# lxtGH/Video-K-Net

Hardware: AMD Instinct MI355X
Metric: frames/sec (S=3, N=100, 1024x2048) (higher is better)
Workload: dtype f32; 1 GPU; cfg2 video_knet_s3_r50: VideoKernelIterHead S=3, N=100 proposals + 17 stuff = 117 kernels, C=256, 1024x2048 frame -> 128x256 stride-8 features, ffn tracking link, x4 bilinear upsample of the final logits; streams_per_gpu=1, parallelism=frame-sharded dp1, x_storage=fp32

## Files before the change

include/vkn.h:

```cpp
#ifndef VKN_H
#define VKN_H
#include <stddef.h>
#include <stdint.h>

#ifdef __cplusplus
extern "C" {
#endif

#define VKN_VERSION 0x000600

#define VKN_OK 0
#define VKN_E_ARG (-1)
#define VKN_E_SHAPE (-2)
#define VKN_E_WORKSPACE (-3)
#define VKN_E_LAUNCH (-4)
#define VKN_E_ALIGN (-5)
#define VKN_E_RANGE (-6)

#define VKN_STATUS_RANGE 1u

#define VKN_FLAG_REF_KERNELS 1u
#define VKN_FLAG_EXACT_GEMM 2u
#define VKN_FLAG_LOGITS_HANDOFF 4u
#define VKN_FLAG_BITS_HANDOFF 16u
#define VKN_X_F32 0
#define VKN_X_F16 1
#define VKN_X_BF16 2
#define VKN_FLAG_X_F16 64u
#define VKN_FLAG_X_BF16 128u
#define VKN_FLAG_CHAIN_LAUNCHES 256u
#define VKN_FLAG_CHAIN_PERSISTENT 512u
#define VKN_FLAG_JOIN_EARLY 32768u
#define VKN_FLAG_LINK_RESERVE 262144u
#define VKN_FLAG_LINK_NO_RESERVE 524288u
#define VKN_FLAG_SCALED_F16 16384u
#define VKN_FLAG_CHAIN_BF16X3 65536u
#define VKN_FLAG_CHAIN_KSPLIT 8192u
#define VKN_FLAG_SERIAL_LINK 32u
#define VKN_FLAG_CLIP_LINK 8u

#define VKN_FLAG_INIT_SEPARATE 131072u
#define VKN_FLAG_PHASE_A 1024u
#define VKN_FLAG_PHASE_B 2048u
#define VKN_FLAG_PHASE_C 4096u
#define VKN_FLAG_PHASE_MASK (VKN_FLAG_PHASE_A | VKN_FLAG_PHASE_B | VKN_FLAG_PHASE_C)

#define VKN_MAX_FCS 4

typedef struct VknDims {
    int B;
    int N;
    int C;
    int H, W;
    int heads;
    int ff;
    int ncls;
// ... 359 lines not shown
```

video-k-net_amd/csrc/vkn_api.hip:

```cpp
#include "../../include/vkn.h"
#include "../../include/vkn_decode.h"
#include "vkn_common.h"
#include "vkn_launch.h"

namespace {

struct Carver {
    char* base;
    size_t off;
    template <class T>
    T* take(size_t n) {
        off = (off + 255) & ~(size_t)255;
        T* p = base ? reinterpret_cast<T*>(base + off) : nullptr;
        off += n * sizeof(T);
        return p;
    }
};

inline bool aligned16(const void* p) { return (reinterpret_cast<uintptr_t>(p) & 15) == 0; }
inline int npt_of(int N) { return (N + 31) / 32 * 32; }

struct StageWs {
    float *part, *cntp, *xraw, *cnt, *xfeat, *params, *inputf, *ig, *ug, *f, *obj1, *qkv, *ao, *obj2, *h, *partial, *t1, *t2,
        *maskfeat, *kb, *kern32, *lq, *lkv, *lobj, *lupd, *lf;
    _Float16 *kfh, *kfl;
    int* status;
};


enum MasksFrom {
    FROM_LOGITS,
    FROM_BITS,
    FROM_GATHERED,
    FROM_XFEAT
};
enum MasksTo {
    TO_LOGITS,
    TO_BITS,
    TO_GATHER,
    TO_KERNELS,
    TO_NONE
};
struct StageCall {
    const VknStageWeights* w = nullptr;
    const float *x = nullptr, *obj_in = nullptr;
    float *obj_out = nullptr, *cls_logits = nullptr, *x_feat_out = nullptr;
    bool cls_sigmoid = false;
    MasksFrom from = FROM_LOGITS;
    const float *masks_in = nullptr, *xfeat_in = nullptr;
    const unsigned* bits_in = nullptr;
    MasksTo to = TO_LOGITS;
    float* masks_out = nullptr;
    unsigned* bits_out = nullptr;
    float *kern_out = nullptr, *kb_out = nullptr;
    hipEvent_t prof0 = nullptr, prof1 = nullptr, obj_ready = nullptr;
    float* up_out = nullptr;
    int up_stride = 0, up_chunk = 0;
    bool* up_done = nullptr;
    int link_reserve = 0;
    const float* prev_obj = nullptr;
    float* track_out = nullptr;
    const VknStageWeights* link_pre = nullptr;
    const float* prev_pre = nullptr;
    const VknStageWeights* link_track = nullptr;
// ... 597 lines not shown
    const bool pre_link = c.link_pre && c.prev_pre;
    const bool need_xfeat = (pre_link && c.link_pre->dyn_w) || (c.link_track && c.track_src == 1) || c.keep_xfeat;
    if (xdt_of(flags) && !chain_only && (ref || (P % 64) != 0)) return VKN_E_SHAPE;
    PrepW pw;
    VKN_TRY(carve_pw(d, w, flags, &pw));
    const bool comp = pw.dynft != nullptr;
    const bool fewrow = comp && chain_ks_ok(d, w, pw, flags, have_cls), persistent = comp && chain_fast_ok(d, w, pw, flags, have_cls);
    const bool fast = fewrow || persistent;

    const bool will_fast = !given_xfeat && persistent && vkn_dbg_env("VKN_CHAIN_TOUCH", 1);
    const void* touch_nx = vkn_dbg_env("VKN_CHAIN_TOUCH", 1) ? c.touch_next : nullptr;
    const size_t touch_nx_bytes = touch_nx ? c.touch_next_bytes : 0;
    if (c.from == FROM_LOGITS || c.from == FROM_BITS)
        VKN_TRY(run_gather(d, c.x, c.masks_in, c.from == FROM_BITS ? c.bits_in : nullptr, s, flags, st, will_fast ? w->prepared : nullptr,
                           will_fast ? w->prepared_bytes : 0));

    float* xfeat = c.x_feat_out ? c.x_feat_out : s.xfeat;
    VknEpi e = mk_epi(d);
    if (given_xfeat) {
        xfeat = const_cast<float*>(c.xfeat_in);
    } else if (has_ft) {
        if (!comp || c.x_feat_out || need_xfeat) {
            e.bias = w->ft_b; e.rowscale = s.cnt; e.out = xfeat; e.ldo = C;
            VKN_TRY(vkn_launch_gemm(s.xraw, nullptr, C, w->ft_w, pw.ft, M, C, C, 1, nullptr, e, st));
        }
    } else {
        if (hipMemcpyAsync(xfeat, s.xraw, (size_t)M * C * sizeof(float), hipMemcpyDeviceToDevice, st) != hipSuccess)
            return VKN_E_LAUNCH;
    }

// ... 344 lines not shown
        return VKN_E_ALIGN;
    const int nstuff = cat_stuff ? ncls - num_thing_classes : 0, N = Np + nstuff;
    if (C % 32 != 0 || C > 256 || Np > 256 || ncls > 256) return VKN_E_SHAPE;
    InitWs s;
    const size_t need = carve_init(B, Np, ncls, C, P, sem && !seg_preds, nullptr, &s);
    if (!ws || ws_bytes < need || !aligned16(ws)) return VKN_E_WORKSPACE;
    carve_init(B, Np, ncls, C, P, sem && !seg_preds, static_cast<char*>(ws), &s);
    hipStream_t st = static_cast<hipStream_t>(stream);
    const bool ref = (flags & VKN_FLAG_REF_KERNELS) != 0, ref_decode = ref || (P & 1);
    const int xdt = xdt_of(flags);
    if (xdt && (ref || (P % 64) != 0 || with_obj == 2)) return VKN_E_SHAPE;
    const size_t xes = xdt ? 2 : 4;

    const bool one_pass = sem && !ref && !xdt && with_obj != 2 && s.ph && !(flags & VKN_FLAG_INIT_SEPARATE) &&
                          vkn_init_pass_supported(Np, ncls, C, P) != 0;
    const float* xf = loc_feats;
    if (one_pass) {
        VKN_TRY(vkn_launch_split_planes(init_w, s.ph, s.pl, 1, Np, C, st));
        VKN_TRY(vkn_launch_split_planes(seg_w, s.ph + (size_t)Np * C, s.pl + (size_t)Np * C, 1, ncls, C, st));
        InitPassArgs a{};
        a.loc = loc_feats; a.sem = sem_feats; a.kh = s.ph; a.kl = s.pl; a.seg_b = seg_b; a.x_out = x_feats; a.masks = mask_preds;
        a.seg = seg_preds; a.bits = with_obj ? s.bits : nullptr; a.thr = thr_logit; a.Np = Np; a.ncls = ncls; a.nth = num_thing_classes;
        a.cat = nstuff > 0 ? 1 : 0; a.N = N; a.C = C; a.P = P; a.npt = npt_of(Np);
        VKN_TRY(vkn_launch_init_pass(a, B, st));
        xf = x_feats;
    } else {
        if (ref_decode) {
            VKN_TRY(vkn_launch_decode_ref_ex(loc_feats, init_w, nullptr, mask_preds, B, Np, C, P, 1, N, st));
        } else {
            VKN_TRY(vkn_launch_split_planes(init_w, s.ih, s.il, 1, Np, C, st));
// ... 15 lines not shown
            }
            if (xdt) VKN_TRY(vkn_launch_add2_half(sem_feats, loc_feats, x_feats, (size_t)B * C * P, xdt, st));
            else VKN_TRY(vkn_launch_add2(sem_feats, loc_feats, x_feats, (size_t)B * C * P, st));
            xf = x_feats;
        } else if (x_feats && x_feats != loc_feats) {
            if (hipMemcpyAsync(x_feats, loc_feats, (size_t)B * C * P * xes, hipMemcpyDeviceToDevice, st) != hipSuccess)
                return VKN_E_LAUNCH;
        }
    }
    const float* obj = nullptr;
    if (with_obj) {
        if (with_obj == 2) {
            if (ref) return VKN_E_SHAPE;
            VKN_TRY(vkn_launch_gather_soft(xf, mask_preds, thr_logit, s.obj, s.cnt, s.part, s.cntp, B, Np, C, P, N, st));
        } else if (ref) VKN_TRY(vkn_launch_gather_ref_ex(xf, mask_preds, thr_logit, s.obj, s.cnt, B, Np, C, P, N, st));
        else if (one_pass) VKN_TRY(vkn_launch_gather_bits(xf, s.bits, s.obj, s.cnt, s.part, s.cntp, B, Np, C, P, st));
        else VKN_TRY(vkn_launch_gather_ex(xf, mask_preds, thr_logit, s.obj, s.cnt, s.part, s.cntp, B, Np, C, P, N, st, xdt));
        obj = s.obj;
    }
    return vkn_launch_init_finish(init_w, obj, seg_w, proposal_feats, B, Np, N, num_thing_classes, C, st);
}

size_t vkn_sizeof_panoptic_cfg(void) { return sizeof(VknPanopticCfg); }

size_t vkn_panoptic_workspace_bytes(const VknPanopticCfg* cfg, int B, int N) {
    if (!cfg || B <= 0 || N <= 0 || cfg->num_proposals > N || cfg->max_per_img <= 0) return 0;
    return vkn_panoptic_ws_bytes(B, cfg->max_per_img + (N - cfg->num_proposals), cfg->Ho, cfg->Wo);
}

int vkn_panoptic_joint_f32(const VknPanopticCfg* cfg, const float* cls_prob, const float* mask_logits, int B, int N, int ncls,
                           int* panoptic_seg, int* info, int* nseg, int* bbox, void* ws, size_t ws_bytes, void* stream) {
    if (!cfg || !cls_prob || !mask_logits || !panoptic_seg || !info || !nseg || B <= 0 || N <= 0 || ncls <= 0) return VKN_E_ARG;
    if (!ws || !aligned16(ws)) return VKN_E_WORKSPACE;
    return vkn_launch_panoptic_joint(cfg, cls_prob, mask_logits, B, N, ncls, panoptic_seg, info, nseg, bbox, ws, ws_bytes,
                                     static_cast<hipStream_t>(stream));
// ... 367 lines not shown
    StageWs s;
    float *mtmp, *otmp, *ctmp;
    unsigned* bits[2];
    const size_t need = carve_head(d, nullptr, &s, &mtmp, &otmp, &ctmp, bits);
    if (!ws || ws_bytes < need || !aligned16(ws)) return VKN_E_WORKSPACE;
    carve_head(d, static_cast<char*>(ws), &s, &mtmp, &otmp, &ctmp, bits);
    hipStream_t st = static_cast<hipStream_t>(stream);
    const bool use_bits = !(flags & (VKN_FLAG_REF_KERNELS | VKN_FLAG_LOGITS_HANDOFF)) && ((d->H * d->W) % 64) == 0;
    const bool use_fused = use_bits && !(flags & VKN_FLAG_BITS_HANDOFF) && vkn_fused_supported(d->C, d->H * d->W);

    const unsigned ph = flags & VKN_FLAG_PHASE_MASK;
    const bool do_a = !ph || (ph & VKN_FLAG_PHASE_A), do_b = !ph || (ph & VKN_FLAG_PHASE_B), do_c = !ph || (ph & VKN_FLAG_PHASE_C);
    if (ph && !(link_pre && (flags & VKN_FLAG_CLIP_LINK) && prev_obj)) return VKN_E_ARG;

    const int link_reserve = (flags & VKN_FLAG_LINK_NO_RESERVE) ? 0 : ((flags & VKN_FLAG_LINK_RESERVE) ? 2 : 1);
    const float* m_in = mask_preds_in;
    const float* o_in = proposal_feats;
    SideStream* joined = nullptr;
    bool up_done = false;
    for (int sidx = 0; sidx < num_stages; ++sidx) {
        const bool last = (sidx == num_stages - 1);
        if (!last && !do_a) {
            const bool to_out_s = ((num_stages - 1 - sidx) & 1) == 0;
            m_in = to_out_s ? mask_preds_out : mtmp;
            o_in = to_out_s ? obj_out : otmp;
            continue;
        }
        const bool to_out = ((num_stages - 1 - sidx) & 1) == 0;
        float* m_out = to_out ? mask_preds_out : mtmp;
        float* o_out = to_out ? obj_out : otmp;
// ... 1 lines not shown
        const bool clip = prev && (flags & VKN_FLAG_CLIP_LINK);
        SideStream* side = (prev && !(flags & VKN_FLAG_SERIAL_LINK)) ? side_stream() : nullptr;
        const bool link_after = clip || side;
        const float* prev_in_stage = link_after ? nullptr : prev;
        const unsigned* b_in = (use_bits && !use_fused && sidx > 0) ? bits[(sidx - 1) & 1] : nullptr;
        unsigned* b_out = (use_bits && !use_fused && !last) ? bits[sidx & 1] : nullptr;
        const float* prev_pre = (last && link_pre) ? prev_obj : nullptr;
        const bool seq = prev_pre && (flags & VKN_FLAG_CLIP_LINK) && (d->B > 1 || ph);
        const VknStageWeights* ltrack = (last && track_out) ? link_track : nullptr;
        StageCall c{};
        c.w = &stages[sidx]; c.x = x; c.obj_in = o_in; c.obj_out = o_out;
        c.cls_logits = last ? cls_prob : ctmp;
        c.cls_sigmoid = last;
        c.from = (use_fused && sidx > 0) ? FROM_GATHERED : (b_in ? FROM_BITS : FROM_LOGITS);
        c.masks_in = m_in; c.bits_in = b_in;
        c.link_pre = prev_pre ? link_pre : nullptr; c.prev_pre = prev_pre;
        c.link_track = ltrack; c.track_src = track_src;
        if (!last && use_fused && !(flags & (VKN_FLAG_CHAIN_LAUNCHES | VKN_FLAG_EXACT_GEMM)) && stages[sidx + 1].prepared) {
            PrepW pwn;
            (void)carve_pw(d, &stages[sidx + 1], flags, &pwn);
            if ((flags & VKN_FLAG_CHAIN_PERSISTENT) || (d->B * d->N + 31) / 32 >= persistent_min_row_tiles(pwn, flags)) {
                if (chain_h2(pwn, flags, false)) {
                    c.touch_next = pwn.h2[VKN_H2_DYNFT];
                    c.touch_next_bytes = (size_t)(reinterpret_cast<const char*>(pwn.h2_scale) - static_cast<const char*>(pwn.h2[VKN_H2_DYNFT]));
                } else {
                    c.touch_next = stages[sidx + 1].prepared;
                    c.touch_next_bytes = stages[sidx + 1].prepared_bytes;
                }
            }
        }
// ... 70 lines not shown
```

video-k-net_amd/csrc/vkn_common.h:

```cpp
#pragma once
#include <hip/hip_runtime.h>
#include <stdint.h>

typedef _Float16 half8 __attribute__((ext_vector_type(8)));
typedef _Float16 half4 __attribute__((ext_vector_type(4)));
typedef float f32x16 __attribute__((ext_vector_type(16)));
typedef float f32x4 __attribute__((ext_vector_type(4)));
typedef float f32x2 __attribute__((ext_vector_type(2)));

#define VKN_WAVE 64

#ifdef VKN_DEBUG
#include <stdlib.h>
static inline int vkn_dbg_env(const char* name, int dflt) {
    const char* e = getenv(name);
    return e ? atoi(e) : dflt;
}
#else
#define vkn_dbg_env(name, dflt) (dflt)
#endif
#ifdef VKN_DEBUG
#define VKN_ABL_IS(param, k) ((param) == (k))
#else
#define VKN_ABL_IS(param, k) false
// ... 40 lines not shown
    VKN_DPP_STEP(fmaxf, v, 0x143, 0xC, ninf);
    return __uint_as_float((unsigned)__builtin_amdgcn_readlane((int)__float_as_uint(v), 63));
}
#undef VKN_DPP_STEP

#define VKN_OK 0
#define VKN_E_ARG (-1)
#define VKN_E_SHAPE (-2)
#define VKN_E_WORKSPACE (-3)
#define VKN_E_LAUNCH (-4)
#define VKN_E_ALIGN (-5)
#define VKN_E_RANGE (-6)
#ifndef VKN_STATUS_RANGE
#define VKN_STATUS_RANGE 1
#endif

static inline int vkn_allow_full_lds(const void* fn, unsigned long long* done_mask) {
    int dev = 0;
    if (hipGetDevice(&dev) != hipSuccess) return -1;
    const unsigned long long bit = 1ull << (dev & 63);
    if (__atomic_load_n(done_mask, __ATOMIC_ACQUIRE) & bit) return 0;
    hipFuncAttributes fa;
    if (hipFuncGetAttributes(&fa, fn) != hipSuccess) return -1;
    const int dyn = 160 * 1024 - (int)fa.sharedSizeBytes;
    if (hipFuncSetAttribute(fn, hipFuncAttributeMaxDynamicSharedMemorySize, dyn) != hipSuccess) return -1;
    __atomic_fetch_or(done_mask, bit, __ATOMIC_RELEASE);
    return 0;
}
#define VKN_ALLOW_FULL_LDS(fn)                                                        \
    do {                                                                              \
// ... 9 lines not shown
```

video-k-net_amd/csrc/vkn_gather.hip:

```cpp
#include "vkn_common.h"
#include "vkn_launch.h"

#define GA_THREADS 512
#define GA_WAVES 8
#define GA_PT 32
#define GA_LDR 40

template <int NB, int BITS, int XH = 0>
__global__ __launch_bounds__(GA_THREADS, 2) void k_gather_mfma(const float* __restrict__ x,
                                                               const float* __restrict__ masks, float thr,
                                                               float* __restrict__ part, float* __restrict__ cntp, int N,
                                                               int NPT, int n0, int C, int P, int px_per_wg,
                                                               long long mask_fs, int ileave, int x_alias) {
    extern __shared__ __attribute__((aligned(16))) char smem[];
    constexpr bool REAL = (BITS == 2 || BITS == 3);
    static_assert(!(XH && REAL), "half-storage x: binary operands only");
    constexpr int XCH = XH ? 2 : 4;
    const int rows_buf = 2 * C + (REAL ? 2 : 1) * NB * 32;
    _Float16* lds = reinterpret_cast<_Float16*>(smem);

    const int b = blockIdx.y, gidx = blockIdx.x, G = gridDim.x;
    const int tid = threadIdx.x, lane = tid & 63;
    const int wave = __builtin_amdgcn_readfirstlane(tid >> 6);
    const int g = lane >> 5, li = lane & 31;
// ... 479 lines not shown
        xraw[((size_t)b * N + n) * C + c] = s;
    }
    if (threadIdx.x == 0) {
        float s = 0.f;
        for (int p = 0; p < P; ++p)
            if (mp[p] >= thr) s += 1.f;
        cnt[(size_t)b * N + n] = s;
    }
}

int vkn_launch_gather_reduce(const float* part, const float* cntp, float* xraw, float* cnt, int B, int N, int C, int G,
                             hipStream_t stream, int* status, const void* touch, size_t touch_bytes) {
    if (touch_bytes >= (1ull << 31)) touch = nullptr;
    hipLaunchKernelGGL(k_gather_reduce, dim3(B * N), dim3(256), 0, stream, part, cntp, xraw, cnt, N, (N + 31) / 32 * 32, C, G, status,
                       static_cast<const char*>(touch), (unsigned)touch_bytes);
    VKN_CHECK_LAUNCH();
    return VKN_OK;
}

int vkn_gather_groups(int B, int P) {
    int wg_per_frame = 256 / (B > 0 ? B : 1);
    if (wg_per_frame < 1) wg_per_frame = 1;
    int px_per_wg = (P + wg_per_frame - 1) / wg_per_frame;
    px_per_wg = (px_per_wg + GA_PT - 1) / GA_PT * GA_PT;
    return (P + px_per_wg - 1) / px_per_wg;
}

int vkn_launch_gather(const float* x, const float* masks, float thr, float* xraw, float* cnt, float* part, float* cntp,
                      int B, int N, int C, int P, hipStream_t stream, int xdt, int* status, const void* touch, size_t touch_bytes) {
    return vkn_launch_gather_ex(x, masks, thr, xraw, cnt, part, cntp, B, N, C, P, N, stream, xdt, status, touch, touch_bytes);
// ... 122 lines not shown
```

video-k-net_amd/csrc/vkn_init.hip:

```cpp
#include <hip/hip_runtime.h>

#include "vkn_common.h"
#include "vkn_launch.h"

__global__ __launch_bounds__(256) void k_add2(const float* __restrict__ a, const float* __restrict__ b,
                                              float* __restrict__ out, size_t n4, size_t n) {
    const size_t stride = (size_t)gridDim.x * blockDim.x;
    for (size_t i = (size_t)blockIdx.x * blockDim.x + threadIdx.x; i < n4; i += stride) {
        const f32x4 va = __builtin_nontemporal_load(reinterpret_cast<const f32x4*>(a) + i);
        const f32x4 vb = __builtin_nontemporal_load(reinterpret_cast<const f32x4*>(b) + i);
        reinterpret_cast<f32x4*>(out)[i] = va + vb;
    }
    for (size_t i = n4 * 4 + (size_t)blockIdx.x * blockDim.x + threadIdx.x; i < n; i += stride) out[i] = a[i] + b[i];
}

int vkn_launch_add2(const float* a, const float* b, float* out, size_t n, hipStream_t st) {
    const bool vec = ((reinterpret_cast<uintptr_t>(a) | reinterpret_cast<uintptr_t>(b) | reinterpret_cast<uintptr_t>(out)) & 15) == 0;
    const size_t n4 = vec ? n / 4 : 0;
    size_t blocks = (n4 + 255) / 256;
    if (blocks > 8192) blocks = 8192;
    if (blocks < 1) blocks = 1;
    hipLaunchKernelGGL(k_add2, dim3((unsigned)blocks), dim3(256), 0, st, a, b, out, n4, n);
    VKN_CHECK_LAUNCH();
    return VKN_OK;
// ... 27 lines not shown
    const bool vec = ((reinterpret_cast<uintptr_t>(a) | reinterpret_cast<uintptr_t>(b) | reinterpret_cast<uintptr_t>(out)) & 15) == 0;
    const size_t n8 = vec ? n / 8 : 0;
    size_t blocks = (n8 + 255) / 256;
    if (blocks > 8192) blocks = 8192;
    if (blocks < 1) blocks = 1;
    const unsigned short *pa = static_cast<const unsigned short*>(a), *pb = static_cast<const unsigned short*>(b);
    unsigned short* po = static_cast<unsigned short*>(out);
    if (xdt == 1) hipLaunchKernelGGL(k_add2h<1>, dim3((unsigned)blocks), dim3(256), 0, st, pa, pb, po, n8, n);
    else hipLaunchKernelGGL(k_add2h<2>, dim3((unsigned)blocks), dim3(256), 0, st, pa, pb, po, n8, n);
    VKN_CHECK_LAUNCH();
    return VKN_OK;
}

__global__ __launch_bounds__(64) void k_init_finish(const float* __restrict__ init_w, const float* __restrict__ obj,
                                                    const float* __restrict__ seg_w, float* __restrict__ out, int Np, int N,
                                                    int nth, int C) {
    const int row = blockIdx.x;
    const int b = row / N, n = row - b * N;
    for (int c = threadIdx.x; c < C; c += 64) {
        float v;
        if (n < Np) {
            v = init_w[(size_t)n * C + c];
            if (obj) v += obj[((size_t)b * Np + n) * C + c];
        } else {
            v = seg_w[(size_t)(nth + n - Np) * C + c];
        }
        out[(size_t)row * C + c] = v;
    }
}

int vkn_launch_init_finish(const float* init_w, const float* obj, const float* seg_w, float* out, int B, int Np, int N, int nth,
                           int C, hipStream_t st) {
    hipLaunchKernelGGL(k_init_finish, dim3(B * N), dim3(64), 0, st, init_w, obj, seg_w, out, Np, N, nth, C);
    VKN_CHECK_LAUNCH();
    return VKN_OK;
}

typedef unsigned int ip_u32x2 __attribute__((ext_vector_type(2)));
#define IP_THREADS 512
#define IP_WAVES 8
#define IP_TILE 64

template <int NB, int SLO>
__device__ __forceinline__ void ip_store_tile(const f32x16 (&acc)[2][NB], const InitPassArgs& A, __amdgpu_buffer_rsrc_t mrs,
                                              __amdgpu_buffer_rsrc_t srs, int p0, int li, int g, int Ntot) {
    int Pq = A.P;
    asm volatile("" : "+s"(Pq));
    const int vst = ((4 * g) * Pq + 2 * li) << 2;
// ... 5 lines not shown
            const int row0 = nb * 32 + (r & 3) + 8 * (r >> 2);
            const ip_u32x2 v = {__float_as_uint(acc[0][nb][r]), __float_as_uint(acc[1][nb][r])};
            if (nb < SLO) {
                __builtin_amdgcn_raw_buffer_store_b64(v, mrs, vst, (row0 * Pq + p0) << 2, 0);
            } else {
                const int row = row0 + 4 * g, j = row - A.Np;
                const int mrow = row < A.Np ? row : ((A.cat && row < Ntot && j >= A.nth) ? A.Np + j - A.nth : -1);
                const unsigned vm = mrow >= 0 ? (unsigned)((mrow * Pq + p0 + 2 * li) << 2) : oor;
                __builtin_amdgcn_raw_buffer_store_b64(v, mrs, (int)vm, 0, 0);
                const unsigned vs = (j >= 0 && row < Ntot) ? (unsigned)((j * Pq + p0 + 2 * li) << 2) : oor;
                __builtin_amdgcn_raw_buffer_store_b64(v, srs, (int)vs, 0, 0);
            }
        }
}

template <int NB>
__device__ __forceinline__ void ip_emit_bits(const f32x16 (&acc)[2][NB], float thr, unsigned* __restrict__ wbase, int NPT, int lane) {
    constexpr int NH = (NB * 32 + 63) / 64;
    int w[2][NH];
#pragma unroll
    for (int t = 0; t < 2; ++t)
#pragma unroll
        for (int h = 0; h < NH; ++h) w[t][h] = 0;
#pragma unroll
    for (int nb = 0; nb < NB; ++nb)
#pragma unroll
        for (int r = 0; r < 16; ++r) {
            const unsigned long long m0 = __ballot(acc[0][nb][r] >= thr);
            const unsigned long long m1 = __ballot(acc[1][nb][r] >= thr);
#pragma unroll
            for (int g = 0; g < 2; ++g) {
                const int row = nb * 32 + (r & 3) + 8 * (r >> 2) + 4 * g;
                const bool mine = lane == (row & 63);
                w[0][row >> 6] = mine ? (int)(unsigned)(m0 >> (32 * g)) : w[0][row >> 6];
                w[1][row >> 6] = mine ? (int)(unsigned)(m1 >> (32 * g)) : w[1][row >> 6];
            }
            __builtin_amdgcn_sched_barrier(0);
        }
#pragma unroll
    for (int t = 0; t < 2; ++t)
#pragma unroll
        for (int h = 0; h < NH; ++h)
            if (h * 64 + lane < NB * 32) wbase[(size_t)t * NPT + h * 64 + lane] = (unsigned)w[t][h];
}

template <int NBL, int SLO, int SHI>
__global__ __launch_bounds__(IP_THREADS, 2) void k_init_pass(const InitPassArgs A) {
    constexpr int NB = (NBL > SHI + 1) ? NBL : SHI + 1;
    extern __shared__ __attribute__((aligned(16))) char smem[];
    const int C = A.C, P = A.P, LDK = C + 8, KS = C >> 4;
    _Float16* ldsH = reinterpret_cast<_Float16*>(smem);
    _Float16* ldsL = ldsH + NB * 32 * LDK;
    float* kbs = reinterpret_cast<float*>(ldsL + NB * 32 * LDK);
    const int b = blockIdx.y, tid = threadIdx.x, lane = tid & 63;
    const int wave = __builtin_amdgcn_readfirstlane(tid >> 6);
    const int g = lane >> 5, li = lane & 31;
    const int Ntot = A.Np + A.ncls;

// ... 109 lines not shown
            half8 ah_ = *reinterpret_cast<const half8*>(ap_);                                                      \
            half8 al_ = *reinterpret_cast<const half8*>(ap_ + NB * 32 * LDK);                                      \
            if (nb >= SLO) { ah_ = thing_row[nb] ? ah_ : hz; al_ = thing_row[nb] ? al_ : hz; }                     \
            IP_MFMA6(ah_, al_, nb);                                                                                \
        }                                                                                                          \
        IP_SPLIT(SR)                                                                                               \
        _Pragma("unroll") for (int nb = SLO; nb <= SHI; ++nb) {                                                    \
            const _Float16* ap_ = ldsH + (nb * 32 + li) * LDK + cb_;                                               \
            half8 ah_ = *reinterpret_cast<const half8*>(ap_);                                                      \
            half8 al_ = *reinterpret_cast<const half8*>(ap_ + NB * 32 * LDK);                                      \
            ah_ = thing_row[nb] ? hz : ah_; al_ = thing_row[nb] ? hz : al_;                                        \
            IP_MFMA6(ah_, al_, nb);                                                                                \
        }                                                                                                          \
        if (++c_ks == KS) {                                                                                        \
            ip_store_tile<NB, SLO>(acc, A, mrs, ers, p0_, li, g, Ntot);                                            \
            if (A.bits) ip_emit_bits<NB>(acc, A.thr, A.bits + ((size_t)b * (P >> 5) + ((p0_ >> 6) << 1)) * A.npt, A.npt, lane); \
            c_ks = 0;                                                                                              \
            ++c_sl;                                                                                                \
        }                                                                                                          \
    } while (0)

    for (int f = 0; f < total; f += 2) {
        IP_LOAD(L1, S1);
        IP_COMPUTE(L0, S0);
        if (f + 1 >= total) break;
        IP_LOAD(L0, S0);
        IP_COMPUTE(L1, S1);
    }
#undef IP_LOAD
#undef IP_SPLIT
#undef IP_MFMA6
// ... 32 lines not shown
```

video-k-net_amd/csrc/vkn_launch.h:

```cpp
#pragma once
#include <hip/hip_runtime.h>
#include <stddef.h>

struct VknEpi {
    const float* bias;
    const float* rowscale;
    const float* bias2;
    const float* resid;
    int ldr;
    const float* ln_w;
    const float* ln_b;
    int ln_from_col;
    float eps;
    int act;
    float* out;
    int ldo;
    const float* dot_vec;
    const float* dot_bias;
    float* dot_out;
    _Float16* plane_hi;
    _Float16* plane_lo;
    int rows_per_frame;
    int NPT;
};
// ... 13 lines not shown
int vkn_gather_groups(int B, int P);
int vkn_launch_gather_ex(const float* x, const float* masks, float thr, float* xraw, float* cnt, float* part, float* cntp,
                         int B, int N, int C, int P, int mask_rows, hipStream_t stream, int xdt = 0, int* status = nullptr,
                         const void* touch = nullptr, size_t touch_bytes = 0);
int vkn_launch_gather_ref_ex(const float* x, const float* masks, float thr, float* xraw, float* cnt, int B, int N, int C,
                             int P, int mask_rows, hipStream_t stream);
int vkn_launch_gather_real(const float* x, const float* a, float* xraw, float* cnt, float* part, float* cntp, int B, int N, int C,
                           int P, int mask_rows, hipStream_t stream, int x_alias = -1, float x_floor = 0.f);
int vkn_launch_gather_soft(const float* x, const float* masks, float thr, float* xraw, float* cnt, float* part, float* cntp, int B,
                           int N, int C, int P, int mask_rows, hipStream_t stream);
int vkn_launch_gather_bits(const float* x, const unsigned* bits, float* xraw, float* cnt, float* part, float* cntp, int B, int N,
                           int C, int P, hipStream_t stream, int xdt = 0, int* status = nullptr, const void* touch = nullptr,
                           size_t touch_bytes = 0);
int vkn_launch_gather_reduce(const float* part, const float* cntp, float* xraw, float* cnt, int B, int N, int C, int G,
                             hipStream_t stream, int* status = nullptr, const void* touch = nullptr, size_t touch_bytes = 0);
int vkn_fused_supported(int C, int P);
int vkn_launch_fused_decode_gather(const float* x, const _Float16* kfh, const _Float16* kfl, const float* kb, float thr,
                                   float* xraw, float* cnt, float* part, float* cntp, int B, int N, int C, int P,
                                   hipStream_t stream, int xdt = 0, int* status = nullptr, const void* touch = nullptr,
                                   size_t touch_bytes = 0);
int vkn_launch_gather(const float* x, const float* masks, float thr, float* xraw, float* cnt, float* part, float* cntp,
                      int B, int N, int C, int P, hipStream_t stream, int xdt = 0, int* status = nullptr, const void* touch = nullptr,
                      size_t touch_bytes = 0);
int vkn_launch_gather_ref(const float* x, const float* masks, float thr, float* xraw, float* cnt, int B, int N, int C,
                          int P, hipStream_t stream);
struct VknDecodeStrides {
    long long plane;
    long long kb;
    long long out;
};
// ... 23 lines not shown
int vkn_launch_add2_half(const void* a, const void* b, void* out, size_t n, int xdt, hipStream_t st);
int vkn_launch_add_rows(const float* a, const float* pos, float* out, size_t rows, int C, int period, hipStream_t st);
struct InitPassArgs {
    const float *loc, *sem;
    const _Float16 *kh, *kl;
    const float* seg_b;
    float *x_out, *masks, *seg;
    unsigned* bits;
    float thr;
    int Np, ncls, nth, cat, N, C, P, px_per_wg;
    int npt;
};
int vkn_init_pass_supported(int Np, int ncls, int C, int P);
int vkn_launch_init_pass(const InitPassArgs& a, int B, hipStream_t st);
int vkn_launch_init_finish(const float* init_w, const float* obj, const float* seg_w, float* out, int B, int Np, int N, int nth,
                           int C, hipStream_t st);
int vkn_launch_ffn_fused(const float* X, int ldx, const void* W1s, const float* b1, const void* W2s, int M, int C, int FF, int HS,
                         float* partial, const VknEpi& epi2, hipStream_t stream);
int vkn_launch_transpose(const float* src, float* dst, int R, int Cc, hipStream_t st);
int vkn_launch_split_w3(const float* W, void* Wp, int Nout, int K, hipStream_t stream);
int vkn_launch_split_w3_t(const float* W, void* Wp, int Nout, int K, hipStream_t stream);
int vkn_launch_ku_mix(const float* params, const float* inputf, const float* ig, const float* ug, const float* no_w,
                      const float* no_b, const float* ino_w, const float* ino_b, float eps, float* f, int M, int C,
                      hipStream_t stream);
int vkn_launch_attn(const float* Q, int ldq, const float* K, const float* V, int ldkv, float* out, int ldo, int B, int Nq,
                    int Nk, int heads, int hd, hipStream_t stream);
int vkn_launch_upsample(const float* in, float* out, int planes, int H, int W, int S, hipStream_t stream, int out_f16 = 0);

struct VknPanopticCfg;
size_t vkn_panoptic_ws_bytes(int B, int K, int Ho, int Wo);
int vkn_launch_panoptic_joint(const VknPanopticCfg* c, const float* cls, const float* masks, int B, int N, int ncls,
// ... 98 lines not shown
```

video-k-net_amd/ops.py:

```python
import ctypes
import struct
import threading

import torch

from . import _lib
from ._lib import VknDims, VknStageWeights, check

_H = _lib.CONSTS
FLAG_REF_KERNELS = _H['VKN_FLAG_REF_KERNELS']
FLAG_EXACT_GEMM = _H['VKN_FLAG_EXACT_GEMM']
FLAG_LOGITS_HANDOFF = _H['VKN_FLAG_LOGITS_HANDOFF']
FLAG_BITS_HANDOFF = _H['VKN_FLAG_BITS_HANDOFF']
FLAG_CHAIN_LAUNCHES = _H['VKN_FLAG_CHAIN_LAUNCHES']
FLAG_CHAIN_PERSISTENT = _H['VKN_FLAG_CHAIN_PERSISTENT']
FLAG_JOIN_EARLY = _H['VKN_FLAG_JOIN_EARLY']
FLAG_LINK_RESERVE = _H['VKN_FLAG_LINK_RESERVE']
FLAG_LINK_NO_RESERVE = _H['VKN_FLAG_LINK_NO_RESERVE']
FLAG_SCALED_F16 = _H['VKN_FLAG_SCALED_F16']
FLAG_CHAIN_BF16X3 = _H['VKN_FLAG_CHAIN_BF16X3']
FLAG_INIT_SEPARATE = _H['VKN_FLAG_INIT_SEPARATE']
FLAG_CHAIN_KSPLIT = _H['VKN_FLAG_CHAIN_KSPLIT']
FLAG_SERIAL_LINK = _H['VKN_FLAG_SERIAL_LINK']

_tls = threading.local()


def _ptr(t):
    return ctypes.c_void_p(t.data_ptr()) if t is not None else ctypes.c_void_p(0)


def _stream():
    return ctypes.c_void_p(torch.cuda.current_stream().cuda_stream)


def _req(t, name):
    if not torch.is_tensor(t) or not t.is_cuda:
        raise _lib.VknLibraryError(f'{name}: expected a CUDA/HIP tensor — the MI355X path has no CPU fallback')
# ... 45 lines not shown
def workspace_generation(device):
    gen = getattr(_tls, 'ws_gen', None) or {}
    return gen.get((device, torch.cuda.current_stream(device).cuda_stream), 0)


def workspace_status(device=None):
    device = torch.device(device if device is not None else torch.cuda.current_device())
    if device.index is None:
        device = torch.device('cuda', torch.cuda.current_device())
    cache = getattr(_tls, 'ws', None) or {}
    buf = cache.get((device, torch.cuda.current_stream(device).cuda_stream))
    if buf is None:
        return
    with torch.cuda.device(device):
        check(_lib.lib().vkn_workspace_status(_ptr(buf), buf.numel(), _stream()))


_THR_CACHE = {}


def thr_logit(hard_mask_thr=0.5):
    key = float(hard_mask_thr)
    if key in _THR_CACHE:
        return _THR_CACHE[key]
    if not 0.0 < key < 1.0:
        raise ValueError('hard_mask_thr must be in (0, 1)')

    def f2o(f):
        u = struct.unpack('<I', struct.pack('<f', f))[0]
        return u ^ 0xFFFFFFFF if u & 0x80000000 else u | 0x80000000
# ... 293 lines not shown
    ws = _workspace(max(L.vkn_stage_workspace_bytes(ctypes.byref(dims)), 256), dev)
    with torch.cuda.device(dev):
        check(L.vkn_stage_chain_f32(ctypes.byref(dims), ctypes.byref(pack.w), _ptr(xf), _ptr(obj_in), _ptr(cls), _ptr(kern), _ptr(kb),
                                    _ptr(obj), _ptr(ws), ws.numel(), flags, _stream()))
    return cls, kern, kb, obj


PHASE_A, PHASE_B, PHASE_C = _H['VKN_FLAG_PHASE_A'], _H['VKN_FLAG_PHASE_B'], _H['VKN_FLAG_PHASE_C']


def head_forward(dims: VknDims, packs, x, proposal_feats, mask_preds, prev_obj=None, upsample_stride=1, want_track=False,
                 want_scaled=True, flags=0, clip_first_prev=None, decode_events=None, link_pre=None, link_track=None, track_src=0,
                 phase=0, out=None):
    (x, xdt), pf, mp = _req_x(x), _req(proposal_feats, 'proposal_feats'), _req(mask_preds, 'mask_preds')
    flags |= (0, FLAG_X_F16, FLAG_X_BF16)[xdt]
    B, N, C, H, W = dims.B, dims.N, dims.C, dims.H, dims.W
    dev = x.device
    L = _lib.lib()
    S = len(packs)
    for p in packs:
        p.ensure_prepared(dims)
    arr = (VknStageWeights * S)(*[p.w for p in packs])
    if out is not None:
        obj, cls, masks, scaled, track = out
        scaled = scaled if (want_scaled and upsample_stride > 1) else None
    else:
        obj = torch.empty((B, N, C), dtype=torch.float32, device=dev)
        cls = torch.empty((B, N, dims.ncls), dtype=torch.float32, device=dev)
        masks = torch.empty((B, N, H, W), dtype=torch.float32, device=dev)
        scaled = None
# ... 113 lines not shown
    return buf


def linear(A, W, bias=None, w_split=None, act=0, ksplit=1):
    A, W = _req(A, 'A'), _req(W, 'W')
    M, K = A.shape
    Nout = W.shape[0]
    out = torch.empty((M, Nout), dtype=torch.float32, device=A.device)
    ws = _workspace(max(ksplit * M * Nout * 4, 256), A.device, scratch=True)
    with torch.cuda.device(A.device):
        check(_lib.lib().vkn_linear_f32(_ptr(A), _ptr(W), _ptr(w_split), _ptr(bias), _ptr(out), M, K, Nout, int(act), int(ksplit),
                                        _ptr(ws), ws.numel(), _stream()))
    return out


def kernel_init(loc_feats, semantic_feats, init_w, seg_w=None, seg_b=None, num_thing_classes=0, cat_stuff_mask=False,
                proposal_feats_with_obj=True, hard_mask_thr=0.5, want_seg_preds=True, flags=0, use_binary=True):
    loc, xdt = _req_x(loc_feats, 'loc_feats')
    flags = int(flags) | {1: FLAG_X_F16, 2: FLAG_X_BF16}.get(xdt, 0)
    B, C, H, W = loc.shape
    P = H * W
    dev = loc.device
    iw = _req(init_w.reshape(init_w.shape[0], -1), 'init_kernels.weight')
    Np = iw.shape[0]
    if iw.shape[1] != C:
        raise ValueError('init_kernels.weight must be [num_proposals, C, 1, 1] (conv_kernel_size == 1)')
    sem = sw = sb = None
    ncls = 0
    if semantic_feats is not None:
        sem, sdt = _req_x(semantic_feats, 'semantic_feats')
        if sem.shape != loc.shape or sdt != xdt:
            raise ValueError('semantic_feats and loc_feats must have the same shape and storage type')
        sw = _req(seg_w.reshape(seg_w.shape[0], -1), 'conv_seg.weight')
        sb = _req(seg_b, 'conv_seg.bias') if seg_b is not None else None
        ncls = sw.shape[0]
    elif cat_stuff_mask:
        raise ValueError('cat_stuff_mask needs the semantic branch')
    nstuff = ncls - num_thing_classes if cat_stuff_mask else 0
    N = Np + nstuff
    L = _lib.lib()
    x_feats = torch.empty_like(loc) if sem is not None else loc
    masks = torch.empty((B, N, H, W), dtype=torch.float32, device=dev)
    seg = torch.empty((B, ncls, H, W), dtype=torch.float32, device=dev) if (sem is not None and want_seg_preds) else None
    prop = torch.empty((B, N, C), dtype=torch.float32, device=dev)
    nb = L.vkn_kernel_init_workspace_bytes(B, Np, ncls, C, P)
    ws = _workspace(max(nb, 256), dev, scratch=True)
    with torch.cuda.device(dev):
        check(L.vkn_kernel_init_f32(_ptr(loc), _ptr(sem), _ptr(iw), _ptr(sw), _ptr(sb), int(num_thing_classes),
                                    int(bool(cat_stuff_mask)), (1 if use_binary else 2) if proposal_feats_with_obj else 0,
                                    thr_logit(hard_mask_thr),
                                    _ptr(x_feats), _ptr(masks), _ptr(seg), _ptr(prop), B, Np, ncls, C, P, _ptr(ws), ws.numel(),
                                    flags, _stream()))
    return prop, x_feats, masks, seg


def panoptic_joint(cls_prob, mask_logits, num_proposals, num_thing_classes, max_per_img, instance_score_thr, overlap_thr,
                   img_shape, batch_input_shape, ori_shape, upsample_stride=1, want_bbox=False):
    cls, m = _req(cls_prob, 'cls_prob'), _req(mask_logits, 'mask_logits')
    B, N, ncls = cls.shape
    if m.shape[0] != B or m.shape[1] != N:
        raise ValueError('cls_prob [B,N,ncls] and mask_logits [B,N,Hm,Wm] disagree')
    Hm, Wm = int(m.shape[2]), int(m.shape[3])
    cfg = _lib.VknPanopticCfg(int(num_proposals), int(num_thing_classes), int(max_per_img), float(instance_score_thr),
                              float(overlap_thr), int(upsample_stride), Hm, Wm, int(batch_input_shape[0]),
                              int(batch_input_shape[1]), int(img_shape[0]), int(img_shape[1]), int(ori_shape[0]),
                              int(ori_shape[1]))
    K = int(max_per_img) + (N - int(num_proposals))
# ... 609 lines not shown
```

Baseline: 10050 frames/s.

## Reuse init-pass gathered sums for first stage instead of regathering masks

During kernel_init, the bit-mask gather now covers all N kernels (proposals plus stuff) and writes the per-kernel feature sums and counts into an extended proposal buffer. The stuff-class bits are remapped with a lane permute so they line up with the stuff kernels. A record attached to the mask tensor, keyed on tensor versions, pointers and threshold, lets the first iterative stage skip its mask-weighted gather over the full feature map. That stage instead copies the precomputed sums through a small kernel. The cost is Python-side validity checks, a larger proposal buffer, and the risk of stale reuse if in-place edits bypass the version checks.

```diff
diff --git a/include/vkn.h b/include/vkn.h
--- a/include/vkn.h
+++ b/include/vkn.h
@@ -18,6 +18,8 @@
 #define VKN_E_RANGE (-6)
 
 #define VKN_STATUS_RANGE 1u
+
+#define VKN_WS_GATHER0_WORD 1
 
 #define VKN_FLAG_REF_KERNELS 1u
 #define VKN_FLAG_EXACT_GEMM 2u
@@ -40,6 +42,7 @@
 #define VKN_FLAG_CLIP_LINK 8u
 
 #define VKN_FLAG_INIT_SEPARATE 131072u
+#define VKN_FLAG_GATHER0 1048576u
 #define VKN_FLAG_PHASE_A 1024u
 #define VKN_FLAG_PHASE_B 2048u
 #define VKN_FLAG_PHASE_C 4096u
diff --git a/video-k-net_amd/csrc/vkn_api.hip b/video-k-net_amd/csrc/vkn_api.hip
--- a/video-k-net_amd/csrc/vkn_api.hip
+++ b/video-k-net_amd/csrc/vkn_api.hip
@@ -20,6 +20,14 @@
 inline bool aligned16(const void* p) { return (reinterpret_cast<uintptr_t>(p) & 15) == 0; }
 inline int npt_of(int N) { return (N + 31) / 32 * 32; }
 
+struct Gather0 {
+    float *sums, *cnt;
+};
+inline Gather0 gather0_of(float* proposal_feats, int B, int N, int C) {
+    const size_t n = (size_t)B * N * C;
+    return Gather0{proposal_feats + n, proposal_feats + 2 * n};
+}
+
 struct StageWs {
     float *part, *cntp, *xraw, *cnt, *xfeat, *params, *inputf, *ig, *ug, *f, *obj1, *qkv, *ao, *obj2, *h, *partial, *t1, *t2,
         *maskfeat, *kb, *kern32, *lq, *lkv, *lobj, *lupd, *lf;
@@ -32,6 +40,7 @@
     FROM_LOGITS,
     FROM_BITS,
     FROM_GATHERED,
+    FROM_GIVEN,
     FROM_XFEAT
 };
 enum MasksTo {
@@ -47,7 +56,7 @@
     float *obj_out = nullptr, *cls_logits = nullptr, *x_feat_out = nullptr;
     bool cls_sigmoid = false;
     MasksFrom from = FROM_LOGITS;
-    const float *masks_in = nullptr, *xfeat_in = nullptr;
+    const float *masks_in = nullptr, *xfeat_in = nullptr, *given_sums = nullptr, *given_cnt = nullptr;
     const unsigned* bits_in = nullptr;
     MasksTo to = TO_LOGITS;
     float* masks_out = nullptr;
@@ -675,6 +684,9 @@
     if (c.from == FROM_LOGITS || c.from == FROM_BITS)
         VKN_TRY(run_gather(d, c.x, c.masks_in, c.from == FROM_BITS ? c.bits_in : nullptr, s, flags, st, will_fast ? w->prepared : nullptr,
                            will_fast ? w->prepared_bytes : 0));
+    else if (c.from == FROM_GIVEN)
+        VKN_TRY(vkn_launch_gather_given(c.given_sums, c.given_cnt, s.xraw, s.cnt, (size_t)M, C, st, s.status, will_fast ? w->prepared : nullptr,
+                                        will_fast ? w->prepared_bytes : 0));
 
     float* xfeat = c.x_feat_out ? c.x_feat_out : s.xfeat;
     VknEpi e = mk_epi(d);
@@ -1049,6 +1061,9 @@
 
     const bool one_pass = sem && !ref && !xdt && with_obj != 2 && s.ph && !(flags & VKN_FLAG_INIT_SEPARATE) &&
                           vkn_init_pass_supported(Np, ncls, C, P) != 0;
+    const bool gather0 = (flags & VKN_FLAG_GATHER0) != 0;
+    if (gather0 && !(one_pass && with_obj == 1 && npt_of(N) == npt_of(Np))) return VKN_E_SHAPE;
+    const Gather0 g0 = gather0_of(proposal_feats, B, N, C);
     const float* xf = loc_feats;
     if (one_pass) {
         VKN_TRY(vkn_launch_split_planes(init_w, s.ph, s.pl, 1, Np, C, st));
@@ -1094,11 +1109,12 @@
             if (ref) return VKN_E_SHAPE;
             VKN_TRY(vkn_launch_gather_soft(xf, mask_preds, thr_logit, s.obj, s.cnt, s.part, s.cntp, B, Np, C, P, N, st));
         } else if (ref) VKN_TRY(vkn_launch_gather_ref_ex(xf, mask_preds, thr_logit, s.obj, s.cnt, B, Np, C, P, N, st));
+        else if (gather0) VKN_TRY(vkn_launch_gather_bits(xf, s.bits, g0.sums, g0.cnt, s.part, s.cntp, B, N, C, P, st));
         else if (one_pass) VKN_TRY(vkn_launch_gather_bits(xf, s.bits, s.obj, s.cnt, s.part, s.cntp, B, Np, C, P, st));
         else VKN_TRY(vkn_launch_gather_ex(xf, mask_preds, thr_logit, s.obj, s.cnt, s.part, s.cntp, B, Np, C, P, N, st, xdt));
-        obj = s.obj;
-    }
-    return vkn_launch_init_finish(init_w, obj, seg_w, proposal_feats, B, Np, N, num_thing_classes, C, st);
+        obj = gather0 ? g0.sums : s.obj;
+    }
+    return vkn_launch_init_finish(init_w, obj, seg_w, proposal_feats, B, Np, N, num_thing_classes, C, st, gather0 ? N : Np);
 }
 
 size_t vkn_sizeof_panoptic_cfg(void) { return sizeof(VknPanopticCfg); }
@@ -1496,6 +1512,8 @@
     if (ph && !(link_pre && (flags & VKN_FLAG_CLIP_LINK) && prev_obj)) return VKN_E_ARG;
 
     const int link_reserve = (flags & VKN_FLAG_LINK_NO_RESERVE) ? 0 : ((flags & VKN_FLAG_LINK_RESERVE) ? 2 : 1);
+    const bool given0 = (flags & VKN_FLAG_GATHER0) && !(flags & VKN_FLAG_REF_KERNELS) && !xdt_of(flags) && !((d->H * d->W) & 1) && do_a;
+    const Gather0 g0 = gather0_of(const_cast<float*>(proposal_feats), d->B, d->N, d->C);
     const float* m_in = mask_preds_in;
     const float* o_in = proposal_feats;
     SideStream* joined = nullptr;
@@ -1527,6 +1545,7 @@
         c.cls_sigmoid = last;
         c.from = (use_fused && sidx > 0) ? FROM_GATHERED : (b_in ? FROM_BITS : FROM_LOGITS);
         c.masks_in = m_in; c.bits_in = b_in;
+        if (given0 && sidx == 0 && !seq) { c.from = FROM_GIVEN; c.given_sums = g0.sums; c.given_cnt = g0.cnt; }
         c.link_pre = prev_pre ? link_pre : nullptr; c.prev_pre = prev_pre;
         c.link_track = ltrack; c.track_src = track_src;
         if (!last && use_fused && !(flags & (VKN_FLAG_CHAIN_LAUNCHES | VKN_FLAG_EXACT_GEMM)) && stages[sidx + 1].prepared) {
diff --git a/video-k-net_amd/csrc/vkn_common.h b/video-k-net_amd/csrc/vkn_common.h
--- a/video-k-net_amd/csrc/vkn_common.h
+++ b/video-k-net_amd/csrc/vkn_common.h
@@ -78,6 +78,9 @@
 #ifndef VKN_STATUS_RANGE
 #define VKN_STATUS_RANGE 1
 #endif
+#ifndef VKN_WS_GATHER0_WORD
+#define VKN_WS_GATHER0_WORD 1
+#endif
 
 static inline int vkn_allow_full_lds(const void* fn, unsigned long long* done_mask) {
     int dev = 0;
diff --git a/video-k-net_amd/csrc/vkn_gather.hip b/video-k-net_amd/csrc/vkn_gather.hip
--- a/video-k-net_amd/csrc/vkn_gather.hip
+++ b/video-k-net_amd/csrc/vkn_gather.hip
@@ -517,6 +517,43 @@
     if (touch_bytes >= (1ull << 31)) touch = nullptr;
     hipLaunchKernelGGL(k_gather_reduce, dim3(B * N), dim3(256), 0, stream, part, cntp, xraw, cnt, N, (N + 31) / 32 * 32, C, G, status,
                        static_cast<const char*>(touch), (unsigned)touch_bytes);
+    VKN_CHECK_LAUNCH();
+    return VKN_OK;
+}
+
+__global__ __launch_bounds__(256) void k_gather_given(const float* __restrict__ sums, const float* __restrict__ counts,
+                                                       float* __restrict__ xraw, float* __restrict__ cnt, unsigned n4, unsigned M,
+                                                       int* __restrict__ status, const char* __restrict__ touch, unsigned touch_bytes) {
+    if (touch) {
+        const unsigned per = (touch_bytes / gridDim.x + 15u) & ~15u;
+        const unsigned t0 = blockIdx.x * per, t1 = min(t0 + per, touch_bytes & ~15u);
+        for (unsigned o = t0 + threadIdx.x * 16u; o < t1; o += 256u * 16u) {
+            const f32x4 v = *reinterpret_cast<const f32x4*>(touch + o);
+            asm volatile("" ::"v"(v));
+        }
+    }
+    const unsigned stride = gridDim.x * 256u, i0 = blockIdx.x * 256u + threadIdx.x;
+    bool bad = false;
+    for (unsigned i = i0; i < n4; i += stride) {
+        const f32x4 r = reinterpret_cast<const f32x4*>(sums)[i];
+        reinterpret_cast<f32x4*>(xraw)[i] = r;
+        bad |= !(fabsf(r[0]) <= 3.0e38f && fabsf(r[1]) <= 3.0e38f && fabsf(r[2]) <= 3.0e38f && fabsf(r[3]) <= 3.0e38f);
+    }
+    for (unsigned i = i0; i < M; i += stride) cnt[i] = counts[i];
+    if (status && bad) atomicOr(status, 1);
+    if (status && i0 == 0) atomicAdd(status + VKN_WS_GATHER0_WORD, 1);
+}
+
+int vkn_launch_gather_given(const float* sums, const float* counts, float* xraw, float* cnt, size_t M, int C, hipStream_t stream,
+                            int* status, const void* touch, size_t touch_bytes) {
+    const size_t n = M * (size_t)C;
+    if (!sums || !counts || !xraw || !cnt || M == 0 || C <= 0 || (n & 3) || n >= ((size_t)1 << 33)) return VKN_E_ARG;
+    if (touch_bytes >= (1ull << 31)) touch = nullptr;
+    size_t blocks = (n / 4 + 255) / 256;
+    if (blocks < 256) blocks = 256;
+    if (blocks > 4096) blocks = 4096;
+    hipLaunchKernelGGL(k_gather_given, dim3((unsigned)blocks), dim3(256), 0, stream, sums, counts, xraw, cnt, (unsigned)(n / 4), (unsigned)M,
+                       status, static_cast<const char*>(touch), touch ? (unsigned)touch_bytes : 0u);
     VKN_CHECK_LAUNCH();
     return VKN_OK;
 }
diff --git a/video-k-net_amd/csrc/vkn_init.hip b/video-k-net_amd/csrc/vkn_init.hip
--- a/video-k-net_amd/csrc/vkn_init.hip
+++ b/video-k-net_amd/csrc/vkn_init.hip
@@ -65,14 +65,14 @@
 
 __global__ __launch_bounds__(64) void k_init_finish(const float* __restrict__ init_w, const float* __restrict__ obj,
                                                     const float* __restrict__ seg_w, float* __restrict__ out, int Np, int N,
-                                                    int nth, int C) {
+                                                    int nth, int C, int obj_rows) {
     const int row = blockIdx.x;
     const int b = row / N, n = row - b * N;
     for (int c = threadIdx.x; c < C; c += 64) {
         float v;
         if (n < Np) {
             v = init_w[(size_t)n * C + c];
-            if (obj) v += obj[((size_t)b * Np + n) * C + c];
+            if (obj) v += obj[((size_t)b * obj_rows + n) * C + c];
         } else {
             v = seg_w[(size_t)(nth + n - Np) * C + c];
         }
@@ -81,8 +81,8 @@
 }
 
 int vkn_launch_init_finish(const float* init_w, const float* obj, const float* seg_w, float* out, int B, int Np, int N, int nth,
-                           int C, hipStream_t st) {
-    hipLaunchKernelGGL(k_init_finish, dim3(B * N), dim3(64), 0, st, init_w, obj, seg_w, out, Np, N, nth, C);
+                           int C, hipStream_t st, int obj_rows) {
+    hipLaunchKernelGGL(k_init_finish, dim3(B * N), dim3(64), 0, st, init_w, obj, seg_w, out, Np, N, nth, C, obj_rows > 0 ? obj_rows : Np);
     VKN_CHECK_LAUNCH();
     return VKN_OK;
 }
@@ -118,9 +118,11 @@
         }
 }
 
-template <int NB>
-__device__ __forceinline__ void ip_emit_bits(const f32x16 (&acc)[2][NB], float thr, unsigned* __restrict__ wbase, int NPT, int lane) {
+template <int NB, int SLO>
+__device__ __forceinline__ void ip_emit_bits(const f32x16 (&acc)[2][NB], const InitPassArgs& A, unsigned* __restrict__ wbase, int lane) {
     constexpr int NH = (NB * 32 + 63) / 64;
+    const float thr = A.thr;
+    const int NPT = A.npt;
     int w[2][NH];
 #pragma unroll
     for (int t = 0; t < 2; ++t)
@@ -144,8 +146,15 @@
 #pragma unroll
     for (int t = 0; t < 2; ++t)
 #pragma unroll
-        for (int h = 0; h < NH; ++h)
-            if (h * 64 + lane < NB * 32) wbase[(size_t)t * NPT + h * 64 + lane] = (unsigned)w[t][h];
+        for (int h = 0; h < NH; ++h) {
+            int v = w[t][h];
+            if (h * 64 + 63 >= SLO * 32) {
+                const int d = h * 64 + lane, src = d < A.Np ? d : d + A.nth;
+                const int got = __builtin_amdgcn_ds_bpermute((src & 63) << 2, v);
+                v = d < A.N ? got : 0;
+            }
+            if (h * 64 + lane < NB * 32) wbase[(size_t)t * NPT + h * 64 + lane] = (unsigned)v;
+        }
 }
 
 template <int NBL, int SLO, int SHI>
@@ -285,7 +294,7 @@
         }                                                                                                          \
         if (++c_ks == KS) {                                                                                        \
             ip_store_tile<NB, SLO>(acc, A, mrs, ers, p0_, li, g, Ntot);                                            \
-            if (A.bits) ip_emit_bits<NB>(acc, A.thr, A.bits + ((size_t)b * (P >> 5) + ((p0_ >> 6) << 1)) * A.npt, A.npt, lane); \
+            if (A.bits) ip_emit_bits<NB, SLO>(acc, A, A.bits + ((size_t)b * (P >> 5) + ((p0_ >> 6) << 1)) * A.npt, lane);      \
             c_ks = 0;                                                                                              \
             ++c_sl;                                                                                                \
         }                                                                                                          \
diff --git a/video-k-net_amd/csrc/vkn_launch.h b/video-k-net_amd/csrc/vkn_launch.h
--- a/video-k-net_amd/csrc/vkn_launch.h
+++ b/video-k-net_amd/csrc/vkn_launch.h
@@ -51,6 +51,8 @@
                            size_t touch_bytes = 0);
 int vkn_launch_gather_reduce(const float* part, const float* cntp, float* xraw, float* cnt, int B, int N, int C, int G,
                              hipStream_t stream, int* status = nullptr, const void* touch = nullptr, size_t touch_bytes = 0);
+int vkn_launch_gather_given(const float* sums, const float* counts, float* xraw, float* cnt, size_t M, int C, hipStream_t stream,
+                            int* status = nullptr, const void* touch = nullptr, size_t touch_bytes = 0);
 int vkn_fused_supported(int C, int P);
 int vkn_launch_fused_decode_gather(const float* x, const _Float16* kfh, const _Float16* kfl, const float* kb, float thr,
                                    float* xraw, float* cnt, float* part, float* cntp, int B, int N, int C, int P,
@@ -104,7 +106,7 @@
 int vkn_init_pass_supported(int Np, int ncls, int C, int P);
 int vkn_launch_init_pass(const InitPassArgs& a, int B, hipStream_t st);
 int vkn_launch_init_finish(const float* init_w, const float* obj, const float* seg_w, float* out, int B, int Np, int N, int nth,
-                           int C, hipStream_t st);
+                           int C, hipStream_t st, int obj_rows = 0);
 int vkn_launch_ffn_fused(const float* X, int ldx, const void* W1s, const float* b1, const void* W2s, int M, int C, int FF, int HS,
                          float* partial, const VknEpi& epi2, hipStream_t stream);
 int vkn_launch_transpose(const float* src, float* dst, int R, int Cc, hipStream_t st);
diff --git a/video-k-net_amd/ops.py b/video-k-net_amd/ops.py
--- a/video-k-net_amd/ops.py
+++ b/video-k-net_amd/ops.py
@@ -1,6 +1,7 @@
 import ctypes
 import struct
 import threading
+import weakref
 
 import torch
 
@@ -22,6 +23,7 @@
 FLAG_INIT_SEPARATE = _H['VKN_FLAG_INIT_SEPARATE']
 FLAG_CHAIN_KSPLIT = _H['VKN_FLAG_CHAIN_KSPLIT']
 FLAG_SERIAL_LINK = _H['VKN_FLAG_SERIAL_LINK']
+FLAG_GATHER0 = _H['VKN_FLAG_GATHER0']
 
 _tls = threading.local()
 
@@ -97,6 +99,17 @@
         return
     with torch.cuda.device(device):
         check(_lib.lib().vkn_workspace_status(_ptr(buf), buf.numel(), _stream()))
+
+
+def workspace_gather0_count(device=None):
+    device = torch.device(device if device is not None else torch.cuda.current_device())
+    if device.index is None:
+        device = torch.device('cuda', torch.cuda.current_device())
+    buf = (getattr(_tls, 'ws', None) or {}).get((device, torch.cuda.current_stream(device).cuda_stream))
+    if buf is None:
+        return 0
+    w = 4 * _H['VKN_WS_GATHER0_WORD']
+    return int(buf[w:w + 4].view(torch.int32).item())
 
 
 _THR_CACHE = {}
@@ -420,6 +433,9 @@
                  phase=0, out=None):
     (x, xdt), pf, mp = _req_x(x), _req(proposal_feats, 'proposal_feats'), _req(mask_preds, 'mask_preds')
     flags |= (0, FLAG_X_F16, FLAG_X_BF16)[xdt]
+    flags &= ~FLAG_GATHER0
+    if mp is mask_preds and gather0_valid(getattr(mask_preds, GATHER0_ATTR, None), mp, x, pf, dims, flags | int(phase)):
+        flags |= FLAG_GATHER0
     B, N, C, H, W = dims.B, dims.N, dims.C, dims.H, dims.W
     dev = x.device
     L = _lib.lib()
@@ -563,6 +579,39 @@
     return out
 
 
+GATHER0_ATTR = '_vkn_gather0'
+_GATHER0_REFUSED = set()
+
+
+class Gather0Record:
+    __slots__ = ('buf', 'sums', 'cnt', 'prop_ptr', 'prop_version', 'x_ptr', 'x_ref', 'x_version', 'm_version', 'thr', 'shape')
+
+    def __init__(self, buf, prop, x_feats, mask_preds, thr, B, N, C, H, W):
+        n = B * N * C
+        self.buf, self.sums, self.cnt = buf, buf[n:2 * n].view(B, N, C), buf[2 * n:].view(B, N)
+        self.prop_ptr, self.prop_version = prop.data_ptr(), prop._version
+        self.x_ptr, self.x_ref, self.x_version = x_feats.data_ptr(), weakref.ref(x_feats), x_feats._version
+        self.m_version, self.thr, self.shape = mask_preds._version, float(thr), (B, N, C, H, W)
+
+
+def gather0_valid(rec, mask_preds, x, proposal_feats, dims, flags):
+    if not isinstance(rec, Gather0Record):
+        return False
+    if flags & (FLAG_REF_KERNELS | FLAG_X_F16 | FLAG_X_BF16) or x.dtype != torch.float32:
+        return False
+    if flags & (PHASE_A | PHASE_B | PHASE_C) and not flags & PHASE_A:
+        return False
+    B, N, C, H, W = rec.shape
+    if (dims.B, dims.N, dims.C, dims.H, dims.W) != rec.shape or (H * W) % 2 or float(dims.thr_logit) != rec.thr:
+        return False
+    if tuple(mask_preds.shape) != (B, N, H, W) or mask_preds._version != rec.m_version:
+        return False
+    if rec.x_ref() is None or x.data_ptr() != rec.x_ptr or x.numel() != B * C * H * W or x._version != rec.x_version:
+        return False
+    return (proposal_feats.data_ptr() == rec.prop_ptr and proposal_feats.numel() == B * N * C
+            and proposal_feats._version == rec.prop_version)
+
+
 def kernel_init(loc_feats, semantic_feats, init_w, seg_w=None, seg_b=None, num_thing_classes=0, cat_stuff_mask=False,
                 proposal_feats_with_obj=True, hard_mask_thr=0.5, want_seg_preds=True, flags=0, use_binary=True):
     loc, xdt = _req_x(loc_feats, 'loc_feats')
@@ -591,15 +640,32 @@
     x_feats = torch.empty_like(loc) if sem is not None else loc
     masks = torch.empty((B, N, H, W), dtype=torch.float32, device=dev)
     seg = torch.empty((B, ncls, H, W), dtype=torch.float32, device=dev) if (sem is not None and want_seg_preds) else None
-    prop = torch.empty((B, N, C), dtype=torch.float32, device=dev)
     nb = L.vkn_kernel_init_workspace_bytes(B, Np, ncls, C, P)
     ws = _workspace(max(nb, 256), dev, scratch=True)
-    with torch.cuda.device(dev):
-        check(L.vkn_kernel_init_f32(_ptr(loc), _ptr(sem), _ptr(iw), _ptr(sw), _ptr(sb), int(num_thing_classes),
-                                    int(bool(cat_stuff_mask)), (1 if use_binary else 2) if proposal_feats_with_obj else 0,
-                                    thr_logit(hard_mask_thr),
-                                    _ptr(x_feats), _ptr(masks), _ptr(seg), _ptr(prop), B, Np, ncls, C, P, _ptr(ws), ws.numel(),
-                                    flags, _stream()))
+    thr = thr_logit(hard_mask_thr)
+    flags &= ~FLAG_GATHER0
+
+    def call(prop, fl):
+        with torch.cuda.device(dev):
+            return L.vkn_kernel_init_f32(_ptr(loc), _ptr(sem), _ptr(iw), _ptr(sw), _ptr(sb), int(num_thing_classes),
+                                         int(bool(cat_stuff_mask)), (1 if use_binary else 2) if proposal_feats_with_obj else 0, thr,
+                                         _ptr(x_feats), _ptr(masks), _ptr(seg), _ptr(prop), B, Np, ncls, C, P, _ptr(ws), ws.numel(),
+                                         fl, _stream())
+    shape_key = (Np, ncls, int(num_thing_classes), bool(cat_stuff_mask), C, P)
+    if (sem is not None and proposal_feats_with_obj and use_binary and xdt == 0 and not flags & (FLAG_REF_KERNELS | FLAG_INIT_SEPARATE)
+            and shape_key not in _GATHER0_REFUSED):
+        n = B * N * C
+        buf = torch.empty(2 * n + B * N, dtype=torch.float32, device=dev)
+        prop = buf[:n].view(B, N, C)
+        code = call(prop, flags | FLAG_GATHER0)
+        if code == 0:
+            setattr(masks, GATHER0_ATTR, Gather0Record(buf, prop, x_feats, masks, thr, B, N, C, H, W))
+            return prop, x_feats, masks, seg
+        if code != _H['VKN_E_SHAPE']:
+            check(code)
+        _GATHER0_REFUSED.add(shape_key)
+    prop = torch.empty((B, N, C), dtype=torch.float32, device=dev)
+    check(call(prop, flags))
     return prop, x_feats, masks, seg
 
 
```

Result: no change. 10080 frames/s (median of 3 runs) (+0.4%).
